# weiguangzhao/PBNet

Hardware: AMD Instinct MI355X
Metric: scenes/sec fwd+cluster (ScanNet ~150k pts/scene) (higher is better)
Workload: dtype bf16; 1 GPU; configs[1]: 1 scene, 161517 pts, 146038 voxels @2cm, 1 rotated copy, full PBNet.forward (MinkUNet34C + grouping + MinkUNet14A mask + MinkUNet34C score); scenes_in_flight_per_gpu=4, scene_seeds=2 (configs[1])

## Files before the change

### pbnet_amd/csrc/cluster.hip

```cpp
#include "pbn_common.h"

#pragma clang fp contract(off)

namespace pbn {
namespace {

constexpr int TPB = 256;
constexpr unsigned long long EMPTY_KEY = ~0ULL;
constexpr int CELL_BIAS = 32768;
constexpr float CELL_CLAMP = 32764.0f;
constexpr int CELL_R = 2;
constexpr int BIG = 0x7f7f7f7f;

__constant__ float c_mean_count[18] = {3917.0f, 12056.0f, 2303.0f, 8331.0f, 3948.0f, 3166.0f, 5629.0f, 11719.0f, 1003.0f,
                                       3317.0f, 4912.0f,  10221.0f, 3889.0f, 4136.0f, 2120.0f, 945.0f,  3967.0f, 2589.0f};

__device__ __forceinline__ float sqdist(float ax, float ay, float az, float bx, float by, float bz) {
    const float dx = __fsub_rn(ax, bx), dy = __fsub_rn(ay, by), dz = __fsub_rn(az, bz);
    const float a = __fmul_rn(dx, dx), b = __fmul_rn(dy, dy), c = __fmul_rn(dz, dz);
    return __fadd_rn(__fadd_rn(a, b), c);
}

__device__ __forceinline__ int cls_of(int sem) { return min(max(sem - 2, 0), 17); }

// ... 114 lines not shown
    const int cx = cell_coord(x, inv_cell), cy = cell_coord(y, inv_cell), cz = cell_coord(z, inv_cell);
    constexpr int W = 2 * CELL_R + 1;
    for (int c = first; c < W * W * W; c += stride) {
        const int dz = c / (W * W) - CELL_R, dy = (c / W) % W - CELL_R, dx = c % W - CELL_R;
        const int slot = hash_lookup(hkeys, hmask, pack_key(seg, cx + dx, cy + dy, cz + dz));
        if (slot < 0) continue;
        const int beg = hstart[slot];
        f(beg, beg + hcount[slot], slot, cell_trusted(cx + dx, cy + dy, cz + dz), (dx | dy | dz) == 0);
    }
}

constexpr int NB_Q = 8;
__device__ __forceinline__ bool group_any(bool pred) {
    const unsigned long long m = __ballot(pred);
    return ((m >> (threadIdx.x & 63 & ~(NB_Q - 1))) & ((1ULL << NB_Q) - 1ULL)) != 0ULL;
}
template <typename F>
__device__ __forceinline__ void for_each_neighbour_cell_group(float x, float y, float z, int seg, float inv_cell,
                                                              const unsigned long long* __restrict__ hkeys, unsigned hmask,
                                                              const int* __restrict__ hstart,
                                                              const int* __restrict__ hcount, int q, F&& f) {
    const int cx = cell_coord(x, inv_cell), cy = cell_coord(y, inv_cell), cz = cell_coord(z, inv_cell);
    constexpr int W = 2 * CELL_R + 1;
    const int gbase = (threadIdx.x & 63) & ~(NB_Q - 1);
    for (int r = 0; r < W * W * W; r += NB_Q) {
        const int c = r + q;
        int slot = -1, beg = 0, end = 0;
        if (c < W * W * W) {
            const int dz = c / (W * W) - CELL_R, dy = (c / W) % W - CELL_R, dx = c % W - CELL_R;
            slot = hash_lookup(hkeys, hmask, pack_key(seg, cx + dx, cy + dy, cz + dz));
            if (slot >= 0) { beg = hstart[slot]; end = beg + hcount[slot]; }
        }
#pragma unroll
        for (int k = 0; k < NB_Q; ++k) {
            const int sk = __shfl(slot, gbase + k, 64);
            if (sk < 0) continue;
            const int bk = __shfl(beg, gbase + k, 64), ek = __shfl(end, gbase + k, 64);
            const int ck = r + k;
            const int dz = ck / (W * W) - CELL_R, dy = (ck / W) % W - CELL_R, dx = ck % W - CELL_R;
            f(bk, ek, sk, cell_trusted(cx + dx, cy + dy, cz + dz), (dx | dy | dz) == 0);
        }
    }
}
__device__ __forceinline__ int group_sum(int v) {
#pragma unroll
    for (int o = 1; o < NB_Q; o <<= 1) v += __shfl_xor(v, o, 64);
    return v;
}
__device__ __forceinline__ int group_max(int v) {
#pragma unroll
    for (int o = 1; o < NB_Q; o <<= 1) v = max(v, __shfl_xor(v, o, 64));
    return v;
}
__global__ __launch_bounds__(TPB) void k_count(const float4* __restrict__ spt, const int* __restrict__ sseg, NRef n_ref,
                                              float inv_cell, float r2, const unsigned long long* __restrict__ hkeys,
                                              unsigned hmask, const int* __restrict__ hstart,
                                              const int* __restrict__ hcount, int* __restrict__ den) {
    __shared__ float4 s_cand[TPB / 64][64];
    const int n = n_ref.get();
    if (n <= 0) return;
    const long long t = (long long)blockIdx.x * TPB + threadIdx.x;
    if ((t - (threadIdx.x & 63)) / NB_Q >= n) return;
    int p = (int)(t / NB_Q);
    const int q = (int)(t % NB_Q);
    const bool live = p < n;
    if (!live) p = n - 1;
    const float4 me = spt[p];
    const int seg = sseg[p];
    const int lane = threadIdx.x & 63, wave = threadIdx.x >> 6;
    const int gbase = lane & ~(NB_Q - 1);
    float4* line = s_cand[wave];
    int cnt = 0;
    const int cx = cell_coord(me.x, inv_cell), cy = cell_coord(me.y, inv_cell), cz = cell_coord(me.z, inv_cell);
    constexpr int W = 2 * CELL_R + 1;
    for (int r = 0; r < W * W * W; r += NB_Q) {
        const int c = r + q;
        int slot = -1, beg = 0, end = 0;
        if (c < W * W * W) {
            const int dz = c / (W * W) - CELL_R, dy = (c / W) % W - CELL_R, dx = c % W - CELL_R;
            slot = hash_lookup(hkeys, hmask, pack_key(seg, cx + dx, cy + dy, cz + dz));
            if (slot >= 0) { beg = hstart[slot]; end = beg + hcount[slot]; }
        }
        const bool same = beg == __shfl(beg, q, 64) && end == __shfl(end, q, 64);
        if (__all(same)) {
#pragma unroll 1
            for (int k = 0; k < NB_Q; ++k) {
                const int bk = __shfl(beg, k, 64), ek = __shfl(end, k, 64);
                float4 nxt = make_float4(0.f, 0.f, 0.f, 0.f);
                if (bk + lane < ek) nxt = spt[bk + lane];
                for (int cb = bk; cb < ek; cb += 64) {
                    line[lane] = nxt;
                    if (cb + 64 + lane < ek) nxt = spt[cb + 64 + lane];
                    const int m = min(64, ek - cb);
#pragma unroll
                    for (int i = 0; i < 64 / NB_Q; ++i) {
                        const int idx = q + NB_Q * i;
                        if (idx < m) {
                            const float4 v = line[idx];
                            cnt += (sqdist(me.x, me.y, me.z, v.x, v.y, v.z) <= r2) ? 1 : 0;
                        }
                    }
                }
            }
        } else {
#pragma unroll
            for (int k = 0; k < NB_Q; ++k) {
                const int sk = __shfl(slot, gbase + k, 64);
                if (sk < 0) continue;
                const int bk = __shfl(beg, gbase + k, 64), ek = __shfl(end, gbase + k, 64);
                int j = bk + q;
                for (; j + NB_Q < ek; j += 2 * NB_Q) {
                    const float4 q0 = spt[j], q1 = spt[j + NB_Q];
                    cnt += (sqdist(me.x, me.y, me.z, q0.x, q0.y, q0.z) <= r2) ? 1 : 0;
                    cnt += (sqdist(me.x, me.y, me.z, q1.x, q1.y, q1.z) <= r2) ? 1 : 0;
                }
                for (; j < ek; j += NB_Q) {
                    const float4 q0 = spt[j];
                    cnt += (sqdist(me.x, me.y, me.z, q0.x, q0.y, q0.z) <= r2) ? 1 : 0;
                }
            }
        }
    }
    cnt = group_sum(cnt);
    if (live && q == 0) den[__float_as_int(me.w)] = cnt - 1;
}

__global__ __launch_bounds__(TPB) void k_tag_hp(float4* __restrict__ spt, NRef n_ref, const int* __restrict__ den, int min_pts,
                                               int* __restrict__ parent, int* __restrict__ lab,
                                               const int* __restrict__ sslot, int* __restrict__ cell_rep) {
    const int n = n_ref.get();
    const int p = blockIdx.x * TPB + threadIdx.x;
    if (p >= n) return;
    const int i = __float_as_int(spt[p].w);
    const int hp = den[i] >= min_pts;
    spt[p].w = __int_as_float(i | (hp ? (int)0x80000000 : 0));
    parent[i] = i;
    lab[i] = -1;
    if (hp) atomicMin(&cell_rep[sslot[p]], i);
}

__device__ __forceinline__ int uf_load(int* p) { return __hip_atomic_load(p, __ATOMIC_RELAXED, __HIP_MEMORY_SCOPE_AGENT); }

__device__ __forceinline__ int uf_find(int* __restrict__ parent, int x) {
    while (true) {
        const int p = uf_load(&parent[x]);
        if (p == x) return x;
        const int gp = uf_load(&parent[p]);
        if (gp == p) return p;
        atomicMin(&parent[x], gp);
        x = gp;
    }
}

__device__ __forceinline__ int uf_union(int* __restrict__ parent, int a, int b) {
    while (true) {
        a = uf_find(parent, a);
        b = uf_find(parent, b);
        if (a == b) return a;
        if (a < b) { const int t = a; a = b; b = t; }
        const int old = atomicMin(&parent[a], b);
        if (old == a) return b;
        a = old;
    }
}

__global__ __launch_bounds__(TPB) void k_union(const float4* __restrict__ spt, const int* __restrict__ sseg, NRef n_ref,
                                              float inv_cell, float r2, const unsigned long long* __restrict__ hkeys,
                                              unsigned hmask, const int* __restrict__ hstart,
                                              const int* __restrict__ hcount, int* parent,
                                              const int* __restrict__ cell_rep, const int* __restrict__ sslot, int pass) {
    const int n = n_ref.get();
    const long long t = (long long)blockIdx.x * TPB + threadIdx.x;
    const int p = (int)(t / NB_Q), q = (int)(t % NB_Q);
    if (p >= n) return;
    const float4 me = spt[p];
    const int wi = __float_as_int(me.w);
    if (wi >= 0) return;
    const int i = wi & 0x7fffffff;
    const int my_rep = cell_rep[sslot[p]];
    const bool own_trusted = cell_trusted(cell_coord(me.x, inv_cell), cell_coord(me.y, inv_cell), cell_coord(me.z, inv_cell));
    int ri = (pass == 0) ? i : parent[i];
    if (pass == 0 && own_trusted) {
        if (my_rep != i) {
            if (q == 0) uf_union(parent, i, my_rep);
            return;
        }
    }
    for_each_neighbour_cell(me.x, me.y, me.z, sseg[p], inv_cell, hkeys, hmask, hstart, hcount, q, NB_Q,
                            [&](int beg, int end, int slot, bool trusted, bool same) {
        const int rep = cell_rep[slot];
        if (rep == BIG) return;
        if (trusted) {
            if (same) return;
            if (rep == ri || parent[rep] == ri) return;
            ri = uf_find(parent, ri);
            if (uf_find(parent, rep) == ri) return;
            for (int j = beg; j < end; ++j) {
                const float4 q = spt[j];
                if (__float_as_int(q.w) < 0 && sqdist(me.x, me.y, me.z, q.x, q.y, q.z) <= r2) {
                    ri = uf_union(parent, ri, __float_as_int(q.w) & 0x7fffffff);
                    return;
                }
            }
            return;
        }
        for (int j = beg; j < end; ++j) {
            const float4 q = spt[j];
            const int wj = __float_as_int(q.w);
            const int jj = wj & 0x7fffffff;
            if (wj < 0 && jj < i && sqdist(me.x, me.y, me.z, q.x, q.y, q.z) <= r2) {
                if (parent[jj] != ri) ri = uf_union(parent, ri, jj);
            }
        }
    });
}

__global__ __launch_bounds__(TPB) void k_compress(const float4* __restrict__ spt, NRef n_ref, int* parent) {
    const int n = n_ref.get();
    const int p = blockIdx.x * TPB + threadIdx.x;
    if (p >= n) return;
    const int wi = __float_as_int(spt[p].w);
    if (wi >= 0) return;
    const int i = wi & 0x7fffffff;
    const int r = uf_find(parent, i);
    if (r != i) atomicMin(&parent[i], r);
}

__global__ __launch_bounds__(TPB) void k_flatten(const float4* __restrict__ spt, NRef n_ref, int* __restrict__ parent,
                                                const int* __restrict__ sem, int general, int* __restrict__ semseed,
                                                int* __restrict__ lab) {
    const int n = n_ref.get();
    const int p = blockIdx.x * TPB + threadIdx.x;
    if (p >= n) return;
    const int wi = __float_as_int(spt[p].w);
    if (wi >= 0) return;
    const int i = wi & 0x7fffffff;
    const int r = uf_find(parent, i);
    lab[i] = r;
    if (general) atomicMin(&semseed[(size_t)cls_of(sem[i]) * n + r], i);
}

__global__ __launch_bounds__(TPB) void k_hp_seed_general(const float4* __restrict__ spt, NRef n_ref, const int* __restrict__ sem,
                                                        const int* __restrict__ semseed, int* __restrict__ lab) {
    const int n = n_ref.get();
    const int p = blockIdx.x * TPB + threadIdx.x;
    if (p >= n) return;
    const int wi = __float_as_int(spt[p].w);
    if (wi >= 0) return;
    const int i = wi & 0x7fffffff;
    lab[i] = semseed[(size_t)cls_of(sem[i]) * n + lab[i]];
}

__global__ __launch_bounds__(TPB) void k_border(const float4* __restrict__ spt, const int* __restrict__ sseg, NRef n_ref,
                                               float inv_cell, float r2, const unsigned long long* __restrict__ hkeys,
                                               unsigned hmask, const int* __restrict__ hstart,
                                               const int* __restrict__ hcount, const int* __restrict__ sem, int general,
                                               const int* __restrict__ semseed, const int* __restrict__ root,
                                               int* __restrict__ lab, const int* __restrict__ cell_rep) {
    const int n = n_ref.get();
    const long long t = (long long)blockIdx.x * TPB + threadIdx.x;
    if (n <= 0 || (t - (threadIdx.x & 63)) / NB_Q >= n) return;
    int p = (int)(t / NB_Q);
    const int q = (int)(t % NB_Q);
    const bool live = p < n;
    if (!live) p = n - 1;
    const float4 me = spt[p];
    const int wi = __float_as_int(me.w);
// ... 246 lines not shown
                const float* v = s_xyz[lane];
                if (fast) {
                    float4 va[4], ya[4], vb[4], yb[4];
                    auto load16 = [&](float4 (&vv)[4], float4 (&yy)[4], int k) {
#pragma unroll
                        for (int q = 0; q < 4; ++q) {
                            vv[q] = *reinterpret_cast<const float4*>(v + k + 4 * q);
                            yy[q] = *reinterpret_cast<const float4*>(s_rcp + k + 4 * q);
                        }
                    };
                    auto chain16 = [&](const float4 (&vv)[4], const float4 (&yy)[4], int k) {
                        const float n0 = (float)(N + k + 1);
                        const int left = cnt - k;
                        if (left >= 16) {
#pragma unroll
                            for (int q = 0; q < 4; ++q) {
                                m = __fadd_rn(m, exact_quotient(__fsub_rn(vv[q].x, m), n0 + (float)(4 * q + 0), yy[q].x));
                                m = __fadd_rn(m, exact_quotient(__fsub_rn(vv[q].y, m), n0 + (float)(4 * q + 1), yy[q].y));
                                m = __fadd_rn(m, exact_quotient(__fsub_rn(vv[q].z, m), n0 + (float)(4 * q + 2), yy[q].z));
                                m = __fadd_rn(m, exact_quotient(__fsub_rn(vv[q].w, m), n0 + (float)(4 * q + 3), yy[q].w));
                            }
                        } else {
                            for (int j = 0; j < left; ++j)
                                m = __fadd_rn(m, exact_quotient(__fsub_rn(v[k + j], m), n0 + (float)j, s_rcp[k + j]));
                        }
                    };
                    load16(va, ya, 0);
                    for (int k = 0; k < cnt; k += 32) {
                        load16(vb, yb, k + 16);
                        chain16(va, ya, k);
                        if (k + 16 < cnt) {
                            load16(va, ya, k + 32);
                            chain16(vb, yb, k + 16);
                        }
                    }
                } else {
                    for (int k = 0; k < cnt; ++k) m = __fadd_rn(m, __fdiv_rn(__fsub_rn(v[k], m), (float)(N + k + 1)));
                }
            }
            N += cnt;
            __syncthreads();
        }
        if (lane < 3) centers[3 * c + lane] = m;
    }
}

__global__ void k_member_tail(int* __restrict__ member_start, const int* __restrict__ total_assigned, int n,
                              const int* __restrict__ n_clusters) {
    if (threadIdx.x == 0 && blockIdx.x == 0) member_start[n] = *total_assigned;
    (void)n_clusters;
}

struct Workspace {
    int *seg_off, *seg_of_pt, *slot_of_pt, *hcount, *hstart, *hcursor, *sseg, *sslot, *cell_rep, *parent, *lab, *root, *semseed, *size,
        *keep, *newid, *lab2, *clt_seg, *last_assigned, *fsize, *noise_flag, *noise_pos, *noise_list, *scan_tmp,
        *scalars, *mstart_tmp;
    unsigned long long* scan_state[4];
    unsigned long long* hkeys;
    float4 *spt, *cand;
    unsigned hcap;
    size_t zero_end, ff_end, big_end;
};

unsigned hash_capacity(int n) {
    unsigned c = 1024;
    while (c < 2u * (unsigned)n) c <<= 1;
    return c;
}

size_t carve(Carver& cv, Workspace& w, int n, int n_seg, int general) {
    const size_t N = (size_t)(n > 0 ? n : 1);
    w.hcap = hash_capacity(n);
    w.scalars = cv.take<int>(64);
    for (int j = 0; j < 4; ++j)
        w.scan_state[j] = cv.take<unsigned long long>(scan_chained_state_words((long long)(w.hcap > N ? w.hcap : N)));
    w.hcount = cv.take<int>(w.hcap);
    w.hcursor = cv.take<int>(w.hcap);
    w.size = cv.take<int>(N);
    w.fsize = cv.take<int>(N);
    w.zero_end = cv.off;
    w.hkeys = cv.take<unsigned long long>(w.hcap);
    w.last_assigned = cv.take<int>((size_t)n_seg + 1);
    w.ff_end = cv.off;
    w.cell_rep = cv.take<int>(w.hcap);
    w.semseed = cv.take<int>(general ? 18 * N : 1);
    w.big_end = cv.off;
    w.hstart = cv.take<int>(w.hcap);
    w.spt = cv.take<float4>(N);
    w.cand = cv.take<float4>(N);
    w.seg_off = cv.take<int>((size_t)n_seg + 1);
    w.seg_of_pt = cv.take<int>(N);
    w.slot_of_pt = cv.take<int>(N);
    w.sseg = cv.take<int>(N);
    w.sslot = cv.take<int>(N);
    w.parent = cv.take<int>(N);
    w.lab = cv.take<int>(N);
    w.root = cv.take<int>(N);
    w.keep = cv.take<int>(N);
    w.newid = cv.take<int>(N);
    w.lab2 = cv.take<int>(N);
    w.clt_seg = cv.take<int>(N);
    w.noise_flag = cv.take<int>(N);
    w.noise_pos = cv.take<int>(N);
    w.noise_list = cv.take<int>(N);
    w.mstart_tmp = cv.take<int>(N + 1);
    w.scan_tmp = cv.take<int>(scan_tmp_ints((long long)(w.hcap > N ? w.hcap : N)));
    return align_up(cv.off, 256);
}

}
}

using namespace pbn;

extern "C" size_t pbn_cluster_workspace_bytes(int n_points, int n_segments, int general_sem) {
    if (n_points < 0 || n_segments < 0) return 0;
    Carver cv(nullptr, 0);
    Workspace w;
    return carve(cv, w, n_points, n_segments, general_sem);
}

extern "C" int pbn_binary_cluster(const float* off_xyz, const float* org_xyz, const int32_t* sem,
                                  const int32_t* seg_len, int n, int n_seg, float radius, int min_pts, float para_f,
                                  int nv_flag, int flags, int32_t* cluster_id, int32_t* cluster_num, int32_t* den,
                                  float* centers, int32_t* clt_sem, int32_t* n_clusters, int32_t* member_start,
                                  int32_t* member_idx, void* workspace, size_t workspace_bytes, pbn_stream_t stream_) {
    hipStream_t stream = (hipStream_t)stream_;
    const int general = flags & 1;
    const int capacity = (flags >> 1) & 1;
    if (n < 0 || n_seg < 0 || n_seg > 65535 || !(radius > 0.0f) || !n_clusters || (n_seg > 0 && !cluster_num))
        return PBN_ERR_ARG;
    if ((member_start == nullptr) != (member_idx == nullptr)) return PBN_ERR_ARG;
    if (n > 0 && (!off_xyz || !org_xyz || !sem || !seg_len || !cluster_id || !den || !centers || !clt_sem || !workspace))
        return PBN_ERR_ARG;
    if (n == 0 || n_seg == 0) {
        if (n_seg > 0) { const int frc_ = fill_bytes(cluster_num, 0, sizeof(int) * (size_t)n_seg, stream); if (frc_ != PBN_OK) return frc_; }
        { const int frc_ = fill_bytes(n_clusters, 0, sizeof(int), stream); if (frc_ != PBN_OK) return frc_; }
        if (member_start) { const int frc_ = fill_bytes(member_start, 0, sizeof(int) * ((size_t)n + 1), stream); if (frc_ != PBN_OK) return frc_; }
        return PBN_OK;
    }
    Carver cv(workspace, workspace_bytes);
    Workspace w;
    carve(cv, w, n, n_seg, general);
    if (!cv.ok) return PBN_ERR_WORKSPACE;

    const float cell = radius * 0.5625f;
    const float inv_cell = 1.0f / cell;
    const float r2 = radius * radius;
    const unsigned hmask = w.hcap - 1;
    const int nb = cdiv(n, TPB);
    const NRef nr{n, capacity ? w.seg_off + n_seg : nullptr};
    int* status = w.scalars + 0;
    int* total_kept = w.scalars + 1;
    int* n_noise = w.scalars + 2;
    int* total_assigned = w.scalars + 3;

    {
        char* base = (char*)workspace;
        char* z0 = (char*)w.scalars;
        char* f0 = (char*)w.hkeys;
        char* b0 = (char*)w.cell_rep;
        FillRange fr[7] = {{cluster_num, sizeof(int) * (size_t)n_seg, 0}, {n_clusters, sizeof(int), 0},
                           {z0, (size_t)(base + w.zero_end - z0), 0}, {f0, (size_t)(base + w.ff_end - f0), 0xff},
                           {b0, (size_t)(base + w.big_end - b0), 0x7f}, {nullptr, 0, 0}, {nullptr, 0, 0}};
        if (capacity) {
            fr[5] = FillRange{w.keep, sizeof(int) * (size_t)n, 0};
            fr[6] = FillRange{w.noise_flag, sizeof(int) * (size_t)n, 0};
        }
        const int frc = fill_ranges(fr, 7, stream);
        if (frc != PBN_OK) return frc;
    }

    hipLaunchKernelGGL(k_seg_offsets, dim3(1), dim3(64), 0, stream, seg_len, n_seg, n, capacity, w.seg_off, status);
    hipLaunchKernelGGL(k_cell_insert, dim3(nb), dim3(TPB), 0, stream, off_xyz, sem, w.seg_off, n_seg, nr, inv_cell,
                       w.hkeys, w.hcount, hmask, w.slot_of_pt, w.seg_of_pt, status);
    int rc = scan_exclusive_i32_chained(w.hcount, w.hstart, (int)w.hcap, w.scan_state[0], nullptr, status, stream);
    if (rc != PBN_OK) return rc;
    hipLaunchKernelGGL(k_cell_scatter, dim3(nb), dim3(TPB), 0, stream, off_xyz, nr, w.slot_of_pt, w.hstart, w.hcursor,
                       w.seg_of_pt, w.spt, w.sseg, w.sslot);
    hipLaunchKernelGGL(k_count, dim3(cdiv((long long)n * NB_Q, TPB)), dim3(TPB), 0, stream, w.spt, w.sseg, nr, inv_cell, r2, w.hkeys, hmask,
                       w.hstart, w.hcount, den);
    hipLaunchKernelGGL(k_tag_hp, dim3(nb), dim3(TPB), 0, stream, w.spt, nr, den, min_pts, w.parent, w.lab, w.sslot, w.cell_rep);
    const dim3 nbq(cdiv((long long)n * NB_Q, TPB));
    hipLaunchKernelGGL(k_union, nbq, dim3(TPB), 0, stream, w.spt, w.sseg, nr, inv_cell, r2, w.hkeys, hmask,
                       w.hstart, w.hcount, w.parent, w.cell_rep, w.sslot, 0);
    hipLaunchKernelGGL(k_compress, dim3(nb), dim3(TPB), 0, stream, w.spt, nr, w.parent);
    hipLaunchKernelGGL(k_union, nbq, dim3(TPB), 0, stream, w.spt, w.sseg, nr, inv_cell, r2, w.hkeys, hmask,
                       w.hstart, w.hcount, w.parent, w.cell_rep, w.sslot, 1);
    hipLaunchKernelGGL(k_flatten, dim3(nb), dim3(TPB), 0, stream, w.spt, nr, w.parent, sem, general, w.semseed, w.lab);
    hipLaunchKernelGGL(k_copy_i32, dim3(nb), dim3(TPB), 0, stream, w.lab, w.root, nr);
    if (general)
        hipLaunchKernelGGL(k_hp_seed_general, dim3(nb), dim3(TPB), 0, stream, w.spt, nr, sem, w.semseed, w.lab);
    hipLaunchKernelGGL(k_border, nbq, dim3(TPB), 0, stream, w.spt, w.sseg, nr, inv_cell, r2, w.hkeys, hmask,
                       w.hstart, w.hcount, sem, general, w.semseed, w.root, w.lab, w.cell_rep);
    hipLaunchKernelGGL(k_sizes, dim3(nb), dim3(TPB), 0, stream, w.lab, nr, w.size);
    hipLaunchKernelGGL(k_keep, dim3(nb), dim3(TPB), 0, stream, w.lab, w.size, sem, nr, para_f, w.keep);
    rc = scan_exclusive_i32_chained(w.keep, w.newid, n, w.scan_state[1], total_kept, status, stream);
    if (rc != PBN_OK) return rc;
    hipLaunchKernelGGL(k_relabel, dim3(nb), dim3(TPB), 0, stream, w.lab, w.keep, w.newid, sem, w.seg_of_pt, org_xyz, nr,
                       w.lab2, cluster_id, clt_sem, w.clt_seg, w.last_assigned, w.fsize, w.noise_flag, w.cand, w.size);
    hipLaunchKernelGGL(k_cluster_num, dim3(cdiv(n_seg, 64)), dim3(64), 0, stream, w.newid, w.seg_off, n_seg, nr,
                       total_kept, cluster_num, status, n_clusters);
    if (nv_flag) {
        rc = scan_exclusive_i32_chained(w.noise_flag, w.noise_pos, n, w.scan_state[2], n_noise, status, stream);
        if (rc != PBN_OK) return rc;
        hipLaunchKernelGGL(k_compact_noise, dim3(nb), dim3(TPB), 0, stream, w.noise_flag, w.noise_pos, nr, w.noise_list);
        hipLaunchKernelGGL(k_noise_nn, dim3(cdiv((long long)n * 64, TPB)), dim3(TPB), 0, stream, w.noise_list, n_noise, w.cand, sem, w.seg_of_pt,
                           w.seg_off, w.lab2, w.last_assigned, cluster_id, w.fsize);
    }
    int* mstart = member_start ? member_start : w.mstart_tmp;
    rc = scan_exclusive_i32_chained(w.fsize, mstart, n, w.scan_state[3], total_assigned, status, stream);
    if (rc != PBN_OK) return rc;
    hipLaunchKernelGGL(k_member_tail, dim3(1), dim3(64), 0, stream, mstart, total_assigned, n, total_kept);
    const int center_blocks = 2048;
    hipLaunchKernelGGL(k_centers, dim3(center_blocks), dim3(CTR_TPB), 0, stream, cluster_id, off_xyz, w.clt_seg, w.seg_off,
                       total_kept, mstart, member_idx, centers);
    PBN_LAUNCH_CHECK();
    return PBN_OK;
}
```

### pbnet_amd/network/PBNet.py

```python
import os
import threading

import numpy as np
import torch
import torch.nn as nn

from .. import MinkowskiEngine as ME
from .. import pbnet_ops
from .. import stage_ops
from ..prof import section, mark
from .Mink import Mink_unet as unet3d

COUNT_MEAN = [-1., -1., 3917., 12056., 2303., 8331., 3948., 3166., 5629., 11719., 1003., 3317., 4912., 10221., 3889.,
              4136., 2120., 945., 3967., 2589.]
LOCAL_VOXEL = 0.02
HEAD_CLUSTERS = 256
MASK_THD = 0.45
TRAIN_FUSED_GLUE = os.environ.get("PBNET_TRAIN_FUSED_GLUE", "1") == "1"
DEVICE_FRONT = os.environ.get("PBNET_DEVICE_FRONT", "1") == "1"
FRONT_CLUSTER_CAP = 1024
FRONT_MAX_POINTS = int(os.environ.get("PBNET_DEVICE_FRONT_MAX_POINTS", "2000000"))


def _mlp(cin, mid, cout, sigmoid=False):
# ... 146 lines not shown
            ins_ind, res, packed, n_ent, n_rows, n_clt, m = front
            n_scenes = n_clt
            with section("a17_gather"), torch.no_grad():
                point_idx, row_scene, coords, feat = stage_ops.local_scene_rows(
                    packed, n_ent, n_rows, res.member_idx, ins_ind, xyz_original, LOCAL_VOXEL, point_feat_p.detach(),
                    sem_sfp.detach(), None)
            self._last_sizes.update(points=int(m), clusters=int(n_clt), entries=int(n_ent), rows=int(n_rows))
            _sec = section("a17_plan"); _sec.__enter__()
        else:
            _sec = section("a6_select"); _sec.__enter__()
            if fused:
                table = s1["table"]
            else:
                batch_head_p = s1["batch_head_p"].long()
                table = torch.bincount(sem_pred_p * nb + batch_head_p, minlength=n_cls * nb)[:n_cls * nb].view(n_cls, nb)
            mark("a6:before table sync")
            tab = table.cpu().numpy()
            mark("a6:table on host")
            assert int(tab.sum()) == sem_pred_p.shape[0], "batch index outside [0, cluster_batch)"
            per_class = tab.sum(1).tolist()
            thr05, thr02 = self._class_thresholds()
            classes = [c for c in range(2, n_cls) if not (float(per_class[c]) < thr05[c])]
            if not classes:
                return self._empty_stage(dev, task)
            m = sum(per_class[c] for c in classes)
            seg_len_h = tab[classes].reshape(-1).astype(np.int32)
            if fused:
                class_base = np.full(n_cls, -1, dtype=np.int32)
                run = 0
                for c in classes:
                    class_base[c] = run
                    run += per_class[c]
                up = torch.from_numpy(np.concatenate([class_base, seg_len_h])).to(dev)
                seg_len = up[n_cls:]
                with torch.no_grad():
                    ins_ind, ins_orig, ins_offseted, ins_sem = stage_ops.select_points(
                        sem_pred_p, up[:n_cls], s1["block_hist"], xyz_original, offset_pred_p.detach(), m)
            else:
                keep = torch.zeros(n_cls, dtype=torch.bool)
                keep[classes] = True
                key = torch.where(keep.to(dev)[sem_pred_p], sem_pred_p, torch.full_like(sem_pred_p, n_cls))
                order = torch.sort(key, stable=True)[1]
                ins_ind = order[:m]
                ins_orig = xyz_original[ins_ind]
                ins_offseted = ins_orig + offset_pred_p[ins_ind].float()
                ins_sem = sem_pred_p[ins_ind].to(torch.int32)
                seg_len = torch.from_numpy(seg_len_h).to(dev)
            _sec.__exit__(None, None, None)

            if fused and not train_glue:
                self._last_sizes["points"] = int(m)
            mark("a7:select queued")
            with section("a7_16_grouping"):
                res = pbnet_ops.cluster_device(ins_offseted, ins_orig, ins_sem, seg_len, self.radius, self.min_pts)
                mark("a7:grouping queued")
                n_seg = int(res.cluster_num.shape[0])
                hc = min(HEAD_CLUSTERS, int(res.member_start.shape[0]) - 1)
                head = torch.cat([res.n_clusters, res.cluster_num, res.member_start[:hc + 1],
                                  res.centers[:3 * hc].view(torch.int32)]).cpu().numpy()
                mark("a7:grouping done")
                n_clt = int(head[0])
            if n_clt < 0:
                raise RuntimeError("grouping rejected its input (class id outside [2,19])")
            if n_clt == 0:
                return self._empty_stage(dev, task)
            _sec = section("a17_plan"); _sec.__enter__()
            cluster_num = head[1:1 + n_seg].reshape(len(classes), nb).tolist()
            if n_clt <= hc:
                member_start = head[1 + n_seg:1 + n_seg + n_clt + 1]
                centers = torch.from_numpy(head[2 + n_seg + hc:2 + n_seg + hc + 3 * n_clt].view(np.float32).copy()).view(n_clt, 3)
            else:
                packed = torch.cat([res.centers[:3 * n_clt], res.member_start[:n_clt + 1].view(torch.float32)]).cpu()
                centers = packed[:3 * n_clt].view(n_clt, 3)
                member_start = packed[3 * n_clt:].view(torch.int32).numpy()
            mark("a17:centres on host")
            sizes = (member_start[1:] - member_start[:-1])
            sizes_l = sizes.tolist()
            labels_h = None
            if task != "test":
                labels_h = ins_label[ins_ind[res.member_idx[:int(member_start[-1])].long()]].cpu()

            ent_cluster, ent_weight, scene_len, scene_gt = [], [], [], []
            k_max = self._k_max_list()
            g = 0
            for ci, cls in enumerate(classes):
                for b in range(nb):
                    c_b = cluster_num[ci][b]
                    if c_b == 0:
                        continue
                    para_k = min(c_b - 1, k_max[cls])
                    if para_k > 0:
                        peak_v = [0.5 * ((para_k + 1) - p_i) / (para_k + 1) for p_i in range(para_k + 1)]
                        ctr = centers[g:g + c_b]
                        knn_idx = torch.cdist(ctr, ctr).topk(k=c_b, dim=1, largest=False)[1].tolist()
                    big = thr02[cls]
                    for c_i in range(c_b):
                        gid = g + c_i
                        gt = None
                        if task != "test":
                            gt = int(torch.mode(labels_h[int(member_start[gid]):int(member_start[gid + 1])])[0])
                            if gt == -100:
                                continue
                        ents, wts = [gid], [1.0]
                        if float(sizes_l[gid]) > big and para_k > 0:
                            row = knn_idx[c_i]
                            for k_i in range(para_k):
                                ents.append(g + row[k_i + 1])
# ... 96 lines not shown
                    iou_feat_f = stage_ops.mlp_rows(self.linear_IOU_feat, *self.score_Unet(inputs_v3).rows())
                    if fused:
                        self._last_sizes["lv3"] = list(inputs_v3.coordinate_manager.row_counts())
                else:
                    iou_feat = self.linear_IOU_feat(self.score_Unet(inputs_v3))
            with section("a20_pool_head"):
                if torch.is_grad_enabled():
                    from ..MinkowskiEngine.nn import global_max_plus_avg_pool
                    global_feat = global_max_plus_avg_pool(iou_feat) if iou_feat.F.is_cuda else \
                        self.global_max_pool(iou_feat) + self.global_avg_pool(iou_feat)
                    out["clt_scores"] = self.linear_IOU(global_feat).F.view(-1)
                else:
                    from ..MinkowskiEngine.nn import segment_pool, _PooledTensor
                    n_prop = int(proposals_offset.shape[0]) - 1
                    f = iou_feat_f if fused_glue else iou_feat.F
                    mx, av = segment_pool(f, inputs_v3.C[:, 0], n_prop)
                    pooled = (mx + av).to(f.dtype)
                    if fused_glue:
                        out["clt_scores"] = stage_ops.mlp_rows(self.linear_IOU, pooled).view(-1)
                    else:
                        out["clt_scores"] = self.linear_IOU(_PooledTensor(pooled)).F.view(-1)
        else:
            out["clt_scores"] = torch.zeros(0, dtype=torch.float32, device=dev)
        mark("a20:score branch queued")
        return out

    def _device_front(self, s1, xyz_original, nb, n_cls):
        from .. import planned as P
        from .. import _native as N
        import ctypes
        dev = xyz_original.device
        lib = N.lib()
        vp = ctypes.c_void_p
        consts = self.__dict__.setdefault("_front_consts", {})
        c = consts.get(dev)
        if c is None:
            thr05, thr02 = self._class_thresholds()
            c = consts[dev] = (torch.tensor(thr05, dtype=torch.float32, device=dev), torch.tensor(thr02, dtype=torch.float32, device=dev),
                               torch.tensor(self._k_max_list(), dtype=torch.int32, device=dev))
        thr05_d, thr02_d, kmax_d = c
        n_pts = int(xyz_original.shape[0])
        n_seg = (n_cls - 2) * nb
        i32 = dict(dtype=torch.int32, device=dev)
        counts = torch.zeros(P.CNT.WORDS, **i32)
        class_base = torch.empty(n_cls, **i32)
        seg_len = torch.empty(n_seg, **i32)
        with section("a6_select"):
            N.check(lib.pbn_class_gate(N.ptr(s1["table"]), N.ptr(thr05_d), n_cls, nb, n_pts, n_pts, N.ptr(class_base), N.ptr(seg_len),
                                       vp(counts.data_ptr()), N.current_stream()), "pbn_class_gate")
            ins_ind, ins_orig, ins_off, ins_sem = stage_ops.select_points(s1["sem_pred_p"], class_base, s1["block_hist"], xyz_original,
                                                                          s1["offset_pred_p"].detach(), n_pts)
        mark("a7:select queued")
        with section("a7_16_grouping"):
            res = pbnet_ops.cluster_device(ins_off, ins_orig, ins_sem, seg_len, self.radius, self.min_pts, capacity=True)
            c_cap = min(FRONT_CLUSTER_CAP, n_pts)
            e_cap = 7 * c_cap
            ent = torch.empty(4 * e_cap + 1, **i32)
            wsb = int(lib.pbn_local_plan_workspace_bytes(c_cap))
            ws = torch.empty(wsb, dtype=torch.uint8, device=dev)
            base = ent.data_ptr()
            N.check(lib.pbn_local_plan(N.ptr(res.cluster_num), n_seg, nb, N.ptr(res.member_start), N.ptr(res.centers),
                                       N.ptr(res.n_clusters), N.ptr(thr02_d), N.ptr(kmax_d), c_cap, e_cap, 2 ** 31 - 1,
                                       vp(base), vp(base + 4 * (e_cap + 1)), vp(base + 4 * (2 * e_cap + 1)),
                                       vp(base + 4 * (3 * e_cap + 1)), vp(counts.data_ptr()), N.ptr(ws), wsb, N.current_stream()),
                    "pbn_local_plan")
            mark("a7:grouping queued")
            h = torch.cat([counts, res.n_clusters]).cpu().tolist()
            mark("a7:grouping done")
        if h[P.CNT.WORDS] < 0:
            raise RuntimeError("grouping rejected its input (class id outside [2,19])")
        if h[P.CNT.OVERFLOW] & 32:
            raise AssertionError("batch index outside [0, cluster_batch)")
        if h[P.CNT.OVERFLOW]:
            return None
        m, n_clt, n_ent, n_rows = h[P.CNT.POINTS], h[P.CNT.CLUSTERS], h[P.CNT.ENTRIES], h[P.CNT.ROWS]
        if m == 0 or n_clt == 0 or n_ent == 0:
            return "empty"
        packed = torch.cat([ent[:n_ent + 1], ent[e_cap + 1:e_cap + 1 + n_ent], ent[2 * e_cap + 1:2 * e_cap + 1 + n_ent],
                            ent[3 * e_cap + 1:3 * e_cap + 1 + n_ent]])
        return ins_ind, res, packed, n_ent, n_rows, n_clt, m

    def _class_thresholds(self):
        hit = getattr(self, "_thr_cache", None)
        if hit is None:
            hit = ((self.count_mean * 0.05).tolist(), (self.count_mean * 0.2).tolist())
            self._thr_cache = hit
        return hit

    def _k_max_list(self):
        hit = getattr(self, "_kmax_cache", None)
        if hit is None:
            hit = [int(v) for v in self.K_max.tolist()]
            self._kmax_cache = hit
        return hit

    def _empty_stage(self, dev, task):
        z = torch.zeros(0, dtype=torch.int64, device=dev)
        out = {"proposals": (torch.zeros(0, 2, dtype=torch.int64, device=dev), torch.zeros(1, dtype=torch.int64, device=dev),
                             z, torch.zeros(0, device=dev)),
               "clt_scores": torch.zeros(0, device=dev)}
        if task != "test":
            out["mask_scores"] = (torch.zeros(0, 1, device=dev), z)
        return out

    def _proposals_fused(self, row_scene, point_idx, mask_score, n_scenes, xyz_original, point_feat_p,
                         mask_score_thd=MASK_THD):
        dev = row_scene.device
# ... 122 lines not shown
```

### pbnet_amd/pbnet_ops.py

```python
import torch
from torch.autograd import Function

from . import _native as N

PARA_F = 0.05
NV_FLAG = True


class ClusterResult(object):
    __slots__ = ("cluster_id", "cluster_num", "den", "centers", "clt_sem", "n_clusters", "member_start",
                 "member_idx")

    def __init__(self, **kw):
        for k, v in kw.items():
            setattr(self, k, v)


def cluster_device(off_xyz, org_xyz, sem, seg_len, radius, min_pts, para_f=PARA_F, nv_flag=NV_FLAG,
                   general_sem=False, want_members=True, capacity=False):
    N.require_cuda(off_xyz, org_xyz, sem, seg_len)
    off_xyz = off_xyz.to(torch.float32).contiguous()
    org_xyz = org_xyz.to(torch.float32).contiguous()
    sem = sem.to(torch.int32).contiguous()
    seg_len = seg_len.to(torch.int32).contiguous()
    n = int(off_xyz.shape[0])
    b = int(seg_len.shape[0])
    dev = off_xyz.device
    i32 = dict(dtype=torch.int32, device=dev)
    cluster_id = torch.empty(n, **i32)
    cluster_num = torch.empty(b, **i32)
    den = torch.empty(n, **i32)
    centers = torch.empty(3 * max(n, 1), dtype=torch.float32, device=dev)
    clt_sem = torch.empty(max(n, 1), **i32)
    n_clusters = torch.empty(1, **i32)
    member_start = torch.empty(n + 1, **i32) if want_members else None
    member_idx = torch.empty(max(n, 1), **i32) if want_members else None
    lib = N.lib()
    ws_bytes = lib.pbn_cluster_workspace_bytes(n, b, int(bool(general_sem)))
    ws = torch.empty(max(ws_bytes, 1), dtype=torch.uint8, device=dev)
    rc = lib.pbn_binary_cluster(N.ptr(off_xyz), N.ptr(org_xyz), N.ptr(sem), N.ptr(seg_len), n, b, float(radius),
                                int(min_pts), float(para_f), int(bool(nv_flag)), int(bool(general_sem)) | (2 if capacity else 0),
                                N.ptr(cluster_id), N.ptr(cluster_num), N.ptr(den), N.ptr(centers), N.ptr(clt_sem),
                                N.ptr(n_clusters), N.ptr(member_start), N.ptr(member_idx), N.ptr(ws), ws_bytes,
                                N.current_stream())
    N.check(rc, "pbn_binary_cluster")
    return ClusterResult(cluster_id=cluster_id, cluster_num=cluster_num, den=den, centers=centers, clt_sem=clt_sem,
                         n_clusters=n_clusters, member_start=member_start, member_idx=member_idx)


class Cluster(Function):

    @staticmethod
    def forward(ctx, ins_offseted, ins_orig, sem, ins_bp, radius, min_pts, batch_size):
        out_dev = ins_offseted.device
        dev = out_dev if out_dev.type == "cuda" else torch.device("cuda", torch.cuda.current_device())
        sem_d = sem.to(dev)
        uniform = True
        if sem_d.numel() > 0:
            uniform = bool((sem_d == sem_d[0]).all().item())
        res = cluster_device(ins_offseted.to(dev), ins_orig.to(dev), sem_d, ins_bp.to(dev)[:batch_size], radius,
                             min_pts, general_sem=not uniform, want_members=False)
        c = int(res.n_clusters.item())
        if c < 0:
            raise RuntimeError("pbnet_ops.cluster: invalid input (segment lengths do not sum to the number of points, "
                               "or a class id outside [2,19])")
        center = res.centers[:3 * c]
        return (res.cluster_id.to(out_dev), res.cluster_num.to(out_dev), (res.den + 1).to(out_dev),
                center.to(out_dev))

    @staticmethod
    def backward(ctx, a=None, b=None, c=None, d=None):
        return None, None, None, None, None, None, None


cluster = Cluster.apply


def get_iou_device(proposals_idx, proposals_offset, instance_labels, instance_pointnum):
    N.require_cuda(proposals_idx, proposals_offset, instance_labels, instance_pointnum)
    n_inst = int(instance_pointnum.size(0))
    n_prop = int(proposals_offset.size(0)) - 1
    idx = proposals_idx.to(torch.int32).contiguous()
    off = proposals_offset.to(torch.int32).contiguous()
    lab = instance_labels.to(torch.int64).contiguous()
    pnum = instance_pointnum.to(torch.int32).contiguous()
    iou = torch.zeros(max(n_prop, 0), n_inst, dtype=torch.float32, device=idx.device)
    rc = N.lib().pbn_get_iou(N.ptr(idx), N.ptr(off), N.ptr(lab), N.ptr(pnum), N.ptr(iou), n_inst, n_prop,
                             N.current_stream())
    N.check(rc, "pbn_get_iou")
    return iou


class GetIoU(Function):

# ... 46 lines not shown
```

### pbnet_amd/planned.py

```python
import ctypes
import os
import sys
from types import SimpleNamespace

import numpy as np
import torch

from . import _native as N
from . import pbnet_ops, stage_ops
from .MinkowskiEngine import conventions as CV
from .MinkowskiEngine.conv import _DT, SPLITK_WORKSPACE_BYTES

CNT = SimpleNamespace(POINTS=0, CLUSTERS=1, ENTRIES=2, ROWS=3, SCENES=4, PROPOSAL_ROWS=5, PROPOSALS=6, OVERFLOW=7, WORDS=16)
OVF_NAMES = {1: "selected points", 2: "clusters", 4: "local-scene entries", 8: "local-scene rows",
             16: "clusters of one (class, batch) segment", 32: "batch index outside [0, cluster_batch)", 64: "rows of a level", 128: "a segment of more than 25 clusters (torch.cdist ranks through its matrix-multiply path: host plan)"}
MASK_THD = 0.45
LOCAL_VOXEL = 0.02
_DEBUG = os.environ.get("PBN_PLANNED_DEBUG", "0") == "1"
HINTS = os.environ.get("PBN_PLANNED_HINTS", "1") != "0"
_STOP = os.environ.get("PBN_PLANNED_STOP", "")


def _dbg(stage, counts=None):
    if _DEBUG:
# ... 118 lines not shown
                                      N.ptr(idx_b), int(n_cap),
                                      vp(n_dev_ptr), N.ptr(hp.w1), N.ptr(hp.scale), N.ptr(hp.shift), N.ptr(hp.slope), hp.hidden,
                                      N.ptr(hp.w2), N.ptr(hp.b2), hp.n_out, int(hp.sigmoid), vp(out.data_ptr()), hp.n_out,
                                      _DT[feats.dtype], N.current_stream())
        N.check(rc, "pbn_mlp_rows_dev")
        return out

    def run(self, feat_voxel, xyz_voxel, xyz_original, v2p_index, teacher=None):
        m, cap, dev, dt, lib = self.model, self.cap, self.dev, self.dtype, N.lib()
        vp = ctypes.c_void_p
        es = torch.empty(0, dtype=dt).element_size()
        n_pts, n_vox, nb = cap.n_points, cap.n_voxels, self.nb
        assert feat_voxel.shape[0] == n_vox and xyz_original.shape[0] == n_pts and feat_voxel.dtype == dt
        self._level_overflow = []
        self._splitk_ws = torch.empty(SPLITK_WORKSPACE_BYTES, dtype=torch.uint8, device=dev)
        counts = torch.zeros(CNT.WORDS, dtype=torch.int32, device=dev)
        cptr = counts.data_ptr()
        cnt = lambda k: cptr + 4 * k
        xyz = xyz_original.float().contiguous()
        st = N.current_stream

        coords1 = xyz_voxel.to(torch.int32).contiguous()
        lin1 = _Lineage(coords1, n_vox, None, dev)
        if _STOP == "prepare1":
            return {"counts": counts, "_keep": {"lin1": lin1, "coords1": coords1}}
        feats1 = feat_voxel.contiguous()
        f = self._unet(m.MEUnet, lin1, cap.lv1, feats1, feats1.shape[1] * es, cap.expect["lv1"])
        _dbg("backbone done", counts)
        if _STOP == "backbone":
            return {"counts": counts, "_keep": {k: v for k, v in locals().items() if torch.is_tensor(v) or isinstance(v, _Lineage)}}
        v2p = v2p_index.long()
        v2p_z = lin1.inv_perm[v2p]
        point_feat_p = f[v2p_z]
        sem_score = stage_ops.mlp_rows(m.linear_sem, f, v2p_z)
        offset_p = stage_ops.mlp_rows(m.linear_offset, f, v2p_z)
        batch_head = coords1[:, 0][v2p]
        if teacher is not None:
            sem_score = teacher["sem_score"].to(dev, sem_score.dtype)
            offset_p = teacher["offset"].to(dev, offset_p.dtype)
        sem_pred, sem_prob, table, block_hist = stage_ops.sem_argmax_table(sem_score, batch_head.contiguous(), nb)
        out = {"sem_pred_p": sem_pred, "sem_pred_score_p": sem_score, "offset_pred_p": offset_p, "counts": counts}

        _dbg("heads done", counts)
        if _STOP == "heads":
            return {"counts": counts, "_keep": {k: v for k, v in locals().items() if torch.is_tensor(v) or isinstance(v, _Lineage)}}
        n_cls = int(m.sem_num)
        n_seg = (n_cls - 2) * nb
        class_base = torch.empty(n_cls, dtype=torch.int32, device=dev)
        seg_len = torch.empty(n_seg, dtype=torch.int32, device=dev)
        N.check(lib.pbn_class_gate(N.ptr(table), N.ptr(self.thr05), n_cls, nb, int(cap.points), n_pts, N.ptr(class_base),
                                   N.ptr(seg_len), vp(cptr), st()), "pbn_class_gate")
        ins_ind, ins_orig, ins_off, ins_sem = stage_ops.select_points(sem_pred, class_base, block_hist, xyz, offset_p,
                                                                      int(cap.points))
        res = pbnet_ops.cluster_device(ins_off, ins_orig, ins_sem, seg_len, m.radius, m.min_pts, capacity=True)

        _dbg("grouping done", counts)
        if _STOP == "grouping":
            return {"counts": counts, "_keep": {k: v for k, v in locals().items() if torch.is_tensor(v) or isinstance(v, _Lineage)}}
        c_cap, e_cap, r_cap = int(cap.clusters), int(cap.entries), int(cap.rows)
        i32 = dict(dtype=torch.int32, device=dev)
        ent_row_start = torch.empty(e_cap + 1, **i32)
        ent_member_start = torch.empty(e_cap, **i32)
        ent_scene = torch.empty(e_cap, **i32)
        ent_weight = torch.empty(e_cap, dtype=torch.float32, device=dev)
        wsb = int(lib.pbn_local_plan_workspace_bytes(c_cap))
        ws = torch.empty(wsb, dtype=torch.uint8, device=dev)
        N.check(lib.pbn_local_plan(N.ptr(res.cluster_num), n_seg, nb, N.ptr(res.member_start), N.ptr(res.centers),
                                   N.ptr(res.n_clusters), N.ptr(self.thr02), N.ptr(self.kmax), c_cap, e_cap, r_cap,
                                   N.ptr(ent_row_start), N.ptr(ent_member_start), N.ptr(ent_scene), N.ptr(ent_weight), vp(cptr),
                                   N.ptr(ws), wsb, st()), "pbn_local_plan")
        c_in = int(point_feat_p.shape[1])
        ld2 = c_in + 2
        point_idx = torch.empty(r_cap, dtype=torch.int64, device=dev)
        row_scene = torch.empty(r_cap, dtype=torch.int64, device=dev)
        coords2 = torch.empty(r_cap, 4, **i32)
        feat2 = torch.empty(r_cap, ld2, dtype=dt, device=dev)
        sem_prob2 = sem_prob.view(-1, 1)
        N.check(lib.pbn_local_scene_rows_dev(
            N.ptr(ent_row_start), N.ptr(ent_member_start), N.ptr(ent_scene), N.ptr(ent_weight), e_cap, r_cap,
            vp(cnt(CNT.ENTRIES)), vp(cnt(CNT.ROWS)), N.ptr(res.member_idx), N.ptr(ins_ind), N.ptr(xyz),
            stage_ops.reciprocal_f32(LOCAL_VOXEL), vp(point_feat_p.data_ptr()), point_feat_p.stride(0), c_in,
            vp(sem_prob2.data_ptr()), sem_prob2.stride(0), None, _DT[dt], N.ptr(point_idx), N.ptr(row_scene), N.ptr(coords2),
            vp(feat2.data_ptr()), ld2, st()), "pbn_local_scene_rows_dev")

        _dbg("local scene rows done", counts)
        if _STOP == "local scene rows":
            return {"counts": counts, "_keep": {k: v for k, v in locals().items() if torch.is_tensor(v) or isinstance(v, _Lineage)}}
        lin2 = _Lineage(coords2, r_cap, cnt(CNT.ROWS), dev)
        f2 = self._unet(m.D_Unet, lin2, cap.lv2, feat2, ld2 * es, cap.expect["lv2"])
        mask_score = self._mlp(m.linear_binary, f2, lin2.inverse, lin2.inv_perm, r_cap, cnt(CNT.ROWS))

        _dbg("mask branch done", counts)
        if _STOP == "mask branch":
            return {"counts": counts, "_keep": {k: v for k, v in locals().items() if torch.is_tensor(v) or isinstance(v, _Lineage)}}
        per_scene = torch.empty(c_cap, **i32)
        block_cnt = torch.empty(max(int(lib.pbn_select_blocks(r_cap)), 1), **i32)
        N.check(lib.pbn_mask_count_dev(vp(mask_score.data_ptr()), 1, float(MASK_THD), N.ptr(row_scene), r_cap, vp(cnt(CNT.ROWS)),
                                       c_cap, _DT[dt], N.ptr(per_scene), N.ptr(block_cnt), st()), "pbn_mask_count_dev")
        proposals_offset = torch.zeros(c_cap + 1, dtype=torch.int64, device=dev)
        alive_ids = torch.zeros(c_cap, dtype=torch.int64, device=dev)
        dense_of = torch.empty(c_cap, **i32)
        N.check(lib.pbn_proposal_offsets(N.ptr(per_scene), c_cap, N.ptr(proposals_offset), N.ptr(alive_ids), N.ptr(dense_of),
                                         vp(cptr), st()), "pbn_proposal_offsets")
        prop_idx = torch.empty(r_cap, 2, dtype=torch.int64, device=dev)
        prop_ms = torch.empty(r_cap, dtype=dt, device=dev)
        coords3 = torch.empty(r_cap, 4, **i32)
        feat3 = torch.empty(r_cap, c_in, dtype=dt, device=dev)
# ... 88 lines not shown
```

Baseline: 348.7 scenes/s.

## Early-exit density counting and skip resolved cells in second union pass

```diff
diff --git a/pbnet_amd/csrc/cluster.hip b/pbnet_amd/csrc/cluster.hip
--- a/pbnet_amd/csrc/cluster.hip
+++ b/pbnet_amd/csrc/cluster.hip
@@ -190,10 +190,18 @@
     for (int o = 1; o < NB_Q; o <<= 1) v = max(v, __shfl_xor(v, o, 64));
     return v;
 }
-__global__ __launch_bounds__(TPB) void k_count(const float4* __restrict__ spt, const int* __restrict__ sseg, NRef n_ref,
-                                              float inv_cell, float r2, const unsigned long long* __restrict__ hkeys,
-                                              unsigned hmask, const int* __restrict__ hstart,
-                                              const int* __restrict__ hcount, int* __restrict__ den) {
+__constant__ unsigned short c_nb_ring[125] = {
+    146, 73,  74,  75,  81,  82,  83,  89,  90,  91,  137, 138, 139, 145, 147, 153, 154, 155, 201, 202, 203, 209, 210, 211, 217,
+    218, 219, 0,   1,   2,   3,   4,   8,   9,   10,  11,  12,  16,  17,  18,  19,  20,  24,  25,  26,  27,  28,  32,  33,  34,
+    35,  36,  64,  65,  66,  67,  68,  72,  76,  80,  84,  88,  92,  96,  97,  98,  99,  100, 128, 129, 130, 131, 132, 136, 140,
+    144, 148, 152, 156, 160, 161, 162, 163, 164, 192, 193, 194, 195, 196, 200, 204, 208, 212, 216, 220, 224, 225, 226, 227, 228,
+    256, 257, 258, 259, 260, 264, 265, 266, 267, 268, 272, 273, 274, 275, 276, 280, 281, 282, 283, 284, 288, 289, 290, 291, 292};
+
+__global__ __launch_bounds__(TPB) void k_count(const float4* __restrict__ spt, const int* __restrict__ sseg,
+                                              const int* __restrict__ sslot, NRef n_ref, float inv_cell, float r2,
+                                              const unsigned long long* __restrict__ hkeys, unsigned hmask,
+                                              const int* __restrict__ hstart, const int* __restrict__ hcount, int min_pts,
+                                              int need_den, int* __restrict__ den) {
     __shared__ float4 s_cand[TPB / 64][64];
     const int n = n_ref.get();
     if (n <= 0) return;
@@ -208,21 +216,26 @@
     const int lane = threadIdx.x & 63, wave = threadIdx.x >> 6;
     const int gbase = lane & ~(NB_Q - 1);
     float4* line = s_cand[wave];
-    int cnt = 0;
     const int cx = cell_coord(me.x, inv_cell), cy = cell_coord(me.y, inv_cell), cz = cell_coord(me.z, inv_cell);
-    constexpr int W = 2 * CELL_R + 1;
-    for (int r = 0; r < W * W * W; r += NB_Q) {
+    const bool own_trusted = cell_trusted(cx, cy, cz);
+    int cnt = (own_trusted && q == 0) ? hcount[sslot[p]] : 0;
+    bool gdone = !live;
+    if (!need_den) gdone = gdone || group_sum(cnt) > min_pts;
+    bool wdone = __all(gdone);
+    constexpr int NCELL = (2 * CELL_R + 1) * (2 * CELL_R + 1) * (2 * CELL_R + 1);
+    for (int r = 0; r < NCELL && !wdone; r += NB_Q) {
         const int c = r + q;
         int slot = -1, beg = 0, end = 0;
-        if (c < W * W * W) {
-            const int dz = c / (W * W) - CELL_R, dy = (c / W) % W - CELL_R, dx = c % W - CELL_R;
+        if (c < NCELL && !gdone && !(c == 0 && own_trusted)) {
+            const int o = c_nb_ring[c];
+            const int dx = (o & 7) - CELL_R, dy = ((o >> 3) & 7) - CELL_R, dz = (o >> 6) - CELL_R;
             slot = hash_lookup(hkeys, hmask, pack_key(seg, cx + dx, cy + dy, cz + dz));
             if (slot >= 0) { beg = hstart[slot]; end = beg + hcount[slot]; }
         }
         const bool same = beg == __shfl(beg, q, 64) && end == __shfl(end, q, 64);
         if (__all(same)) {
 #pragma unroll 1
-            for (int k = 0; k < NB_Q; ++k) {
+            for (int k = 0; k < NB_Q && !wdone; ++k) {
                 const int bk = __shfl(beg, k, 64), ek = __shfl(end, k, 64);
                 float4 nxt = make_float4(0.f, 0.f, 0.f, 0.f);
                 if (bk + lane < ek) nxt = spt[bk + lane];
@@ -238,13 +251,18 @@
                             cnt += (sqdist(me.x, me.y, me.z, v.x, v.y, v.z) <= r2) ? 1 : 0;
                         }
                     }
+                    if (!need_den) {
+                        gdone = gdone || group_sum(cnt) > min_pts;
+                        wdone = __all(gdone);
+                        if (wdone) break;
+                    }
                 }
             }
         } else {
 #pragma unroll
             for (int k = 0; k < NB_Q; ++k) {
                 const int sk = __shfl(slot, gbase + k, 64);
-                if (sk < 0) continue;
+                if (sk < 0 || gdone) continue;
                 const int bk = __shfl(beg, gbase + k, 64), ek = __shfl(end, gbase + k, 64);
                 int j = bk + q;
                 for (; j + NB_Q < ek; j += 2 * NB_Q) {
@@ -256,11 +274,13 @@
                     const float4 q0 = spt[j];
                     cnt += (sqdist(me.x, me.y, me.z, q0.x, q0.y, q0.z) <= r2) ? 1 : 0;
                 }
+                if (!need_den) gdone = group_sum(cnt) > min_pts;
             }
+            wdone = __all(gdone);
         }
     }
     cnt = group_sum(cnt);
-    if (live && q == 0) den[__float_as_int(me.w)] = cnt - 1;
+    if (live && q == 0) den[__float_as_int(me.w)] = need_den ? cnt - 1 : min(cnt - 1, min_pts);
 }
 
 __global__ __launch_bounds__(TPB) void k_tag_hp(float4* __restrict__ spt, NRef n_ref, const int* __restrict__ den, int min_pts,
@@ -302,11 +322,14 @@
     }
 }
 
+template <int PASS>
 __global__ __launch_bounds__(TPB) void k_union(const float4* __restrict__ spt, const int* __restrict__ sseg, NRef n_ref,
                                               float inv_cell, float r2, const unsigned long long* __restrict__ hkeys,
                                               unsigned hmask, const int* __restrict__ hstart,
                                               const int* __restrict__ hcount, int* parent,
-                                              const int* __restrict__ cell_rep, const int* __restrict__ sslot, int pass) {
+                                              const int* __restrict__ cell_rep, const int* __restrict__ sslot,
+                                              int* __restrict__ unres) {
+    constexpr int pass = PASS;
     const int n = n_ref.get();
     const long long t = (long long)blockIdx.x * TPB + threadIdx.x;
     const int p = (int)(t / NB_Q), q = (int)(t % NB_Q);
@@ -315,8 +338,11 @@
     const int wi = __float_as_int(me.w);
     if (wi >= 0) return;
     const int i = wi & 0x7fffffff;
-    const int my_rep = cell_rep[sslot[p]];
+    const int my_slot = sslot[p];
     const bool own_trusted = cell_trusted(cell_coord(me.x, inv_cell), cell_coord(me.y, inv_cell), cell_coord(me.z, inv_cell));
+    if (pass == 1 && own_trusted && !unres[my_slot]) return;
+    const int my_rep = cell_rep[my_slot];
+    bool unresolved = false;
     int ri = (pass == 0) ? i : parent[i];
     if (pass == 0 && own_trusted) {
         if (my_rep != i) {
@@ -333,15 +359,23 @@
             if (rep == ri || parent[rep] == ri) return;
             ri = uf_find(parent, ri);
             if (uf_find(parent, rep) == ri) return;
-            for (int j = beg; j < end; ++j) {
-                const float4 q = spt[j];
-                if (__float_as_int(q.w) < 0 && sqdist(me.x, me.y, me.z, q.x, q.y, q.z) <= r2) {
-                    ri = uf_union(parent, ri, __float_as_int(q.w) & 0x7fffffff);
-                    return;
+            constexpr int WIT = PASS == 0 ? 8 : 1;
+            for (int j = beg; j < end; j += WIT) {
+                float4 c[WIT];
+#pragma unroll
+                for (int u = 0; u < WIT; ++u) c[u] = (j + u < end) ? spt[j + u] : make_float4(0.f, 0.f, 0.f, 0.f);
+#pragma unroll
+                for (int u = 0; u < WIT; ++u) {
+                    if (__float_as_int(c[u].w) < 0 && sqdist(me.x, me.y, me.z, c[u].x, c[u].y, c[u].z) <= r2) {
+                        ri = uf_union(parent, ri, __float_as_int(c[u].w) & 0x7fffffff);
+                        return;
+                    }
                 }
             }
+            unresolved = true;
             return;
         }
+        unresolved = true;
         for (int j = beg; j < end; ++j) {
             const float4 q = spt[j];
             const int wj = __float_as_int(q.w);
@@ -351,6 +385,7 @@
             }
         }
     });
+    if (pass == 0 && own_trusted && unresolved) unres[my_slot] = 1;
 }
 
 __global__ __launch_bounds__(TPB) void k_compress(const float4* __restrict__ spt, NRef n_ref, int* parent) {
@@ -703,7 +738,7 @@
 }
 
 struct Workspace {
-    int *seg_off, *seg_of_pt, *slot_of_pt, *hcount, *hstart, *hcursor, *sseg, *sslot, *cell_rep, *parent, *lab, *root, *semseed, *size,
+    int *seg_off, *seg_of_pt, *slot_of_pt, *hcount, *hstart, *hcursor, *unres, *sseg, *sslot, *cell_rep, *parent, *lab, *root, *semseed, *size,
         *keep, *newid, *lab2, *clt_seg, *last_assigned, *fsize, *noise_flag, *noise_pos, *noise_list, *scan_tmp,
         *scalars, *mstart_tmp;
     unsigned long long* scan_state[4];
@@ -727,6 +762,7 @@
         w.scan_state[j] = cv.take<unsigned long long>(scan_chained_state_words((long long)(w.hcap > N ? w.hcap : N)));
     w.hcount = cv.take<int>(w.hcap);
     w.hcursor = cv.take<int>(w.hcap);
+    w.unres = cv.take<int>(w.hcap);
     w.size = cv.take<int>(N);
     w.fsize = cv.take<int>(N);
     w.zero_end = cv.off;
@@ -779,6 +815,7 @@
     hipStream_t stream = (hipStream_t)stream_;
     const int general = flags & 1;
     const int capacity = (flags >> 1) & 1;
+    const int need_den = !((flags >> 2) & 1);
     if (n < 0 || n_seg < 0 || n_seg > 65535 || !(radius > 0.0f) || !n_clusters || (n_seg > 0 && !cluster_num))
         return PBN_ERR_ARG;
     if ((member_start == nullptr) != (member_idx == nullptr)) return PBN_ERR_ARG;
@@ -829,15 +866,15 @@
     if (rc != PBN_OK) return rc;
     hipLaunchKernelGGL(k_cell_scatter, dim3(nb), dim3(TPB), 0, stream, off_xyz, nr, w.slot_of_pt, w.hstart, w.hcursor,
                        w.seg_of_pt, w.spt, w.sseg, w.sslot);
-    hipLaunchKernelGGL(k_count, dim3(cdiv((long long)n * NB_Q, TPB)), dim3(TPB), 0, stream, w.spt, w.sseg, nr, inv_cell, r2, w.hkeys, hmask,
-                       w.hstart, w.hcount, den);
+    hipLaunchKernelGGL(k_count, dim3(cdiv((long long)n * NB_Q, TPB)), dim3(TPB), 0, stream, w.spt, w.sseg, w.sslot, nr, inv_cell, r2,
+                       w.hkeys, hmask, w.hstart, w.hcount, min_pts, need_den, den);
     hipLaunchKernelGGL(k_tag_hp, dim3(nb), dim3(TPB), 0, stream, w.spt, nr, den, min_pts, w.parent, w.lab, w.sslot, w.cell_rep);
     const dim3 nbq(cdiv((long long)n * NB_Q, TPB));
-    hipLaunchKernelGGL(k_union, nbq, dim3(TPB), 0, stream, w.spt, w.sseg, nr, inv_cell, r2, w.hkeys, hmask,
-                       w.hstart, w.hcount, w.parent, w.cell_rep, w.sslot, 0);
+    hipLaunchKernelGGL(k_union<0>, nbq, dim3(TPB), 0, stream, w.spt, w.sseg, nr, inv_cell, r2, w.hkeys, hmask,
+                       w.hstart, w.hcount, w.parent, w.cell_rep, w.sslot, w.unres);
     hipLaunchKernelGGL(k_compress, dim3(nb), dim3(TPB), 0, stream, w.spt, nr, w.parent);
-    hipLaunchKernelGGL(k_union, nbq, dim3(TPB), 0, stream, w.spt, w.sseg, nr, inv_cell, r2, w.hkeys, hmask,
-                       w.hstart, w.hcount, w.parent, w.cell_rep, w.sslot, 1);
+    hipLaunchKernelGGL(k_union<1>, nbq, dim3(TPB), 0, stream, w.spt, w.sseg, nr, inv_cell, r2, w.hkeys, hmask,
+                       w.hstart, w.hcount, w.parent, w.cell_rep, w.sslot, w.unres);
     hipLaunchKernelGGL(k_flatten, dim3(nb), dim3(TPB), 0, stream, w.spt, nr, w.parent, sem, general, w.semseed, w.lab);
     hipLaunchKernelGGL(k_copy_i32, dim3(nb), dim3(TPB), 0, stream, w.lab, w.root, nr);
     if (general)
diff --git a/pbnet_amd/network/PBNet.py b/pbnet_amd/network/PBNet.py
--- a/pbnet_amd/network/PBNet.py
+++ b/pbnet_amd/network/PBNet.py
@@ -222,7 +222,8 @@
                 self._last_sizes["points"] = int(m)
             mark("a7:select queued")
             with section("a7_16_grouping"):
-                res = pbnet_ops.cluster_device(ins_offseted, ins_orig, ins_sem, seg_len, self.radius, self.min_pts)
+                res = pbnet_ops.cluster_device(ins_offseted, ins_orig, ins_sem, seg_len, self.radius, self.min_pts,
+                                              need_den=False)
                 mark("a7:grouping queued")
                 n_seg = int(res.cluster_num.shape[0])
                 hc = min(HEAD_CLUSTERS, int(res.member_start.shape[0]) - 1)
@@ -425,7 +426,8 @@
                                                                           s1["offset_pred_p"].detach(), n_pts)
         mark("a7:select queued")
         with section("a7_16_grouping"):
-            res = pbnet_ops.cluster_device(ins_off, ins_orig, ins_sem, seg_len, self.radius, self.min_pts, capacity=True)
+            res = pbnet_ops.cluster_device(ins_off, ins_orig, ins_sem, seg_len, self.radius, self.min_pts, capacity=True,
+                                          need_den=False)
             c_cap = min(FRONT_CLUSTER_CAP, n_pts)
             e_cap = 7 * c_cap
             ent = torch.empty(4 * e_cap + 1, **i32)
diff --git a/pbnet_amd/pbnet_ops.py b/pbnet_amd/pbnet_ops.py
--- a/pbnet_amd/pbnet_ops.py
+++ b/pbnet_amd/pbnet_ops.py
@@ -17,7 +17,7 @@
 
 
 def cluster_device(off_xyz, org_xyz, sem, seg_len, radius, min_pts, para_f=PARA_F, nv_flag=NV_FLAG,
-                   general_sem=False, want_members=True, capacity=False):
+                   general_sem=False, want_members=True, capacity=False, need_den=True):
     N.require_cuda(off_xyz, org_xyz, sem, seg_len)
     off_xyz = off_xyz.to(torch.float32).contiguous()
     org_xyz = org_xyz.to(torch.float32).contiguous()
@@ -39,7 +39,7 @@
     ws_bytes = lib.pbn_cluster_workspace_bytes(n, b, int(bool(general_sem)))
     ws = torch.empty(max(ws_bytes, 1), dtype=torch.uint8, device=dev)
     rc = lib.pbn_binary_cluster(N.ptr(off_xyz), N.ptr(org_xyz), N.ptr(sem), N.ptr(seg_len), n, b, float(radius),
-                                int(min_pts), float(para_f), int(bool(nv_flag)), int(bool(general_sem)) | (2 if capacity else 0),
+                                int(min_pts), float(para_f), int(bool(nv_flag)), int(bool(general_sem)) | (2 if capacity else 0) | (0 if need_den else 4),
                                 N.ptr(cluster_id), N.ptr(cluster_num), N.ptr(den), N.ptr(centers), N.ptr(clt_sem),
                                 N.ptr(n_clusters), N.ptr(member_start), N.ptr(member_idx), N.ptr(ws), ws_bytes,
                                 N.current_stream())
diff --git a/pbnet_amd/planned.py b/pbnet_amd/planned.py
--- a/pbnet_amd/planned.py
+++ b/pbnet_amd/planned.py
@@ -194,7 +194,8 @@
                                    N.ptr(seg_len), vp(cptr), st()), "pbn_class_gate")
         ins_ind, ins_orig, ins_off, ins_sem = stage_ops.select_points(sem_pred, class_base, block_hist, xyz, offset_p,
                                                                       int(cap.points))
-        res = pbnet_ops.cluster_device(ins_off, ins_orig, ins_sem, seg_len, m.radius, m.min_pts, capacity=True)
+        res = pbnet_ops.cluster_device(ins_off, ins_orig, ins_sem, seg_len, m.radius, m.min_pts, capacity=True,
+                                      need_den=False)
 
         _dbg("grouping done", counts)
         if _STOP == "grouping":
```

Result: faster. 374.3 scenes/s (median of 6 runs) (+7.4%).
